# cts198859/deeprl_signal_control

Hardware: AMD Instinct MI355X
Metric: env-steps/s (agents x envs x sim-steps/s), large_grid MA2C (higher is better)
Workload: dtype f32; 1 GPU; large_grid 5x5 (25 agents), MA2C LSTM policy (neighbour fingerprint gather), 1024 env instances per GPU; step = 120 control steps (x5 sim-steps) of every instance + 1 A2C update (BPTT, clip, RMSProp); envs_per_gpu=1024, n_step=120, agents=25, parallelism=env-sharded x1, live_vehicles=window mean over the timed region

## Files before the change

deeprl_signal_control_amd/csrc/tsc_model.hip:

```cpp
#include "tsc_common.h"
#include "tsc_gemm.h"
#include "../../include/tsc.h"

#include <cstdlib>
#include <type_traits>
#include <vector>

namespace {

using tsc::f32x16;
using tsc::f32x4;
using tsc::GemmArgs;

constexpr int kOut = 8;
constexpr int kL = 64;
constexpr int kG4 = 4 * kL;

struct Layout {
    int G, A, SMAX, AMAX, H;
    int NZ, fc;
    long long stride, oW1, ob1, oWx, oWh, obl, oWo, obo;
};

__device__ __forceinline__ float sigmoidf_(float x) {
// ... 805 lines not shown
#pragma unroll
        for (int k = 0; k < kOut; ++k) {
            const float pj = __shfl(pim, row0 + k, 64);
            if (k < na) sacc += (double)pj;
            if (k == km) mine = sacc;
        }
        const long long idx = (long long)(e0 + hr) * lay.A + a;
        const double uu = uniform01(seed, step, (unsigned long long)idx);
        const bool below = hc < 8 && km < na && uu < mine / sacc;
        const unsigned long long bal = __ballot(below);
        const unsigned rowbits = (unsigned)((bal >> row0) & 0xFFull);
        const int ans = rowbits ? __ffs((int)rowbits) - 1 : na - 1;
        if (e0 + hr < E) {
            if (hc < 8 && km < lay.AMAX) pi_out[idx * lay.AMAX + km] = pim;
            if (hc == 0) {
                v_out[idx] = vv + hbv;
                if (action_out) action_out[idx] = ans;
            }
        }
    }
}


constexpr int kXLd = 68;
constexpr size_t policy_fwd_fused_lds(int H) { return sizeof(float) * ((size_t)(H + 64) * kXLd + kL * kOut + kOut + 8); }

__global__ void __launch_bounds__(256, 2)
policy_fwd_fused_kernel(const float *__restrict__ params, Layout lay, const int *__restrict__ n_act,
                        const float *__restrict__ obs, const uint8_t *__restrict__ done, float *state, int advance,
                        int E, int n_tiles, float *__restrict__ pi_out, float *__restrict__ v_out, int *action_out,
                        unsigned long long seed, unsigned long long step, long long *dbg,
                        int tslot, long long Ntot, float *X1c, float *Zc, float *Hhc, float *Ccc, float *Hpc,
                        const float *__restrict__ Wg) {
    extern __shared__ __attribute__((aligned(16))) char smem_raw[];
    float *XH = (float *)smem_raw;
    const bool stamp = dbg && blockIdx.x == 8 && threadIdx.x == 0;
    int nstamp = 0;
#define FSTAMP() do { if (stamp) dbg[nstamp++] = clock64(); } while (0)
    if (dbg && threadIdx.x == 0) dbg[64 + 2 * blockIdx.x] = wall_clock64();
    FSTAMP();
    const int b = blockIdx.x, xcd = b & 7, sidx = b >> 3;
    const int g = xcd + 8 * (sidx / n_tiles), tile = sidx % n_tiles;
    if (g >= lay.G) return;
    const int a = g >> 1, tower = g & 1, e0 = tile * 64, H = lay.H, SMAX = lay.SMAX;
    float *Hs = XH + H * kXLd;
    const float *P = params + (long long)g * lay.stride;
    const int tid = threadIdx.x, lane = tid & 63, wave = tid >> 6, li = lane & 31, kh = lane >> 5;

    const int r0 = 32 * (wave & 1), j0 = 32 * (wave >> 1), j = j0 + li;
    const int q4 = SMAX >> 2, AS = lay.A * SMAX, nct = H >> 5;
    const float *W1 = P + lay.oW1, *b1 = P + lay.ob1;
    float4 ov[4];
    int om[4], ok4[4];
#pragma unroll
    for (int q = 0; q < 4; ++q) {
        int idx = tid + 256 * q;
        om[q] = -1;
        if (idx < 64 * q4) om[q] = idx / q4; else idx = 64 * q4 - 1;
        const int m = idx / q4;
        ok4[q] = (idx % q4) * 4;
        const int e = e0 + m < E ? e0 + m : E - 1;
        ov[q] = *reinterpret_cast<const float4 *>(obs + (long long)e * AS + a * SMAX + ok4[q]);
    }
    float bw0[32];
    {
        const int ct = wave < nct ? wave : nct - 1;
        const unsigned wb = (unsigned)(ct * 32 + li) * 4u;
#pragma unroll
        for (int s2 = 0; s2 < 32; ++s2) {
            const int kr = 2 * s2 + kh < SMAX ? 2 * s2 + kh : SMAX - 1;
            bw0[s2] = ldg(W1, wb + (unsigned)(kr * H) * 4u);
        }
    }
    float *WoS = XH + (H + 64) * kXLd;
    if (tid < (kL * kOut + kOut) / 4)
        *reinterpret_cast<float4 *>(WoS + 4 * tid) = *reinterpret_cast<const float4 *>(P + lay.oWo + 4 * tid);
    float c[16], h0v[16];
    int erow[16];
    {
        const float *stb = state + (long long)g * E * 2 * kL;
#pragma unroll
        for (int r = 0; r < 16; ++r) {
            erow[r] = r0 + (r & 3) + 8 * (r >> 2) + 4 * kh;
            const int e = e0 + erow[r] < E ? e0 + erow[r] : E - 1;
            const float keep = 1.0f - (float)done[e];
            const unsigned ob = (unsigned)(e * 2 * kL + j) * 4u;
            c[r] = ldg(stb, ob) * keep; h0v[r] = ldg(stb, ob + kL * 4u) * keep;
        }
    }
#pragma unroll
    for (int q = 0; q < 4; ++q)
        if (om[q] >= 0) {
            Hs[(ok4[q] + 0) * kXLd + om[q]] = ov[q].x; Hs[(ok4[q] + 1) * kXLd + om[q]] = ov[q].y;
            Hs[(ok4[q] + 2) * kXLd + om[q]] = ov[q].z; Hs[(ok4[q] + 3) * kXLd + om[q]] = ov[q].w;
        }
    for (int idx = tid; idx < (64 - SMAX) * 64; idx += 256) Hs[(SMAX + (idx >> 6)) * kXLd + (idx & 63)] = 0.f;
    __syncthreads();
    FSTAMP();
    {
        float bw1[32];
        {
            const int ct = wave + 4 < nct ? wave + 4 : nct - 1;
            const unsigned wb = (unsigned)(ct * 32 + li) * 4u;
#pragma unroll
            for (int s2 = 0; s2 < 32; ++s2) {
                const int kr = 2 * s2 + kh < SMAX ? 2 * s2 + kh : SMAX - 1;
                bw1[s2] = ldg(W1, wb + (unsigned)(kr * H) * 4u);
            }
        }
        auto tile = [&](const float *bw, int ct) {
            f32x16 acc0, acc1;
#pragma unroll
            for (int r = 0; r < 16; ++r) { acc0[r] = 0.f; acc1[r] = 0.f; }
            const int col = ct * 32 + li;
#pragma unroll
            for (int s2 = 0; s2 < 32; ++s2) {
                const float a0 = Hs[(2 * s2 + kh) * kXLd + li], a1 = Hs[(2 * s2 + kh) * kXLd + 32 + li];
                acc0 = __builtin_amdgcn_mfma_f32_32x32x2f32(a0, bw[s2], acc0, 0, 0, 0);
                acc1 = __builtin_amdgcn_mfma_f32_32x32x2f32(a1, bw[s2], acc1, 0, 0, 0);
            }
            const float bias = b1[col];
            int eb1 = e0;
            asm volatile("" : "+v"(eb1));
#pragma unroll
            for (int r = 0; r < 16; ++r) {
                const int row = (r & 3) + 8 * (r >> 2) + 4 * kh;
                float v0 = acc0[r] + bias, v1 = acc1[r] + bias;
                v0 = v0 > 0.f ? v0 : 0.f; v1 = v1 > 0.f ? v1 : 0.f;
                XH[col * kXLd + row] = v0;
                XH[col * kXLd + 32 + row] = v1;
                if (tslot >= 0) {
                    const long long nb = (long long)g * Ntot + (long long)tslot * E + eb1;
                    if (eb1 + row < E) st_stream(X1c + ((nb + row) * H + col), v0);
                    if (eb1 + 32 + row < E) st_stream(X1c + ((nb + 32 + row) * H + col), v1);
                }
            }
        };
        if (wave < nct) tile(bw0, wave);
        if (wave + 4 < nct) tile(bw1, wave + 4);
    }
    __syncthreads();
    FSTAMP();
    int eb15 = e0;
    asm volatile("" : "+v"(eb15));
#pragma unroll
    for (int r = 0; r < 16; ++r) {
        Hs[j * kXLd + erow[r]] = h0v[r];
        if (tslot >= 0 && eb15 + erow[r] < E)
            st_stream(Hpc + (((long long)g * Ntot + (long long)tslot * E + eb15 + erow[r]) * kL + j), h0v[r]);
    }
    __syncthreads();
    FSTAMP();
    f32x16 acc[4];
    {
        const float *bl = P + lay.obl;
#pragma unroll
        for (int q = 0; q < 4; ++q) {
            const float bv = bl[64 * q + j];
#pragma unroll
            for (int r = 0; r < 16; ++r) acc[q][r] = bv;
        }
        const float *B = Wg + (long long)g * (H + 64) * kG4;
        constexpr int CS = 8;
        const int nchunk = (H + 64) / (2 * CS);
        const unsigned bb = (unsigned)(kh * kG4 + 4 * j) * 4u;
        float bA[CS][4], bB[CS][4];
        auto loadB = [&](float (*dst)[4], int chunk) {
            const float *src = B + (long long)chunk * (2 * CS * kG4);
#pragma unroll
            for (int s2 = 0; s2 < CS; ++s2) {
                const float4 w4 = ldg((const float4 *)src, bb + s2 * (2u * kG4 * 4u));
                dst[s2][0] = w4.x; dst[s2][1] = w4.y; dst[s2][2] = w4.z; dst[s2][3] = w4.w;
            }
        };
        auto compute = [&](float (*bv)[4], int chunk) {
            const float *As = XH + (chunk * 2 * CS + kh) * kXLd + r0 + li;
#pragma unroll
            for (int s2 = 0; s2 < CS; ++s2) {
                const float av = As[(2 * s2) * kXLd];
#pragma unroll
                for (int q = 0; q < 4; ++q) acc[q] = __builtin_amdgcn_mfma_f32_32x32x2f32(av, bv[s2][q], acc[q], 0, 0, 0);
            }
        };
        loadB(bA, 0);
        for (int ch = 0; ch < nchunk; ch += 2) {
            loadB(bB, ch + 1);
            compute(bA, ch);
            loadB(bA, ch + 2 < nchunk ? ch + 2 : nchunk - 1);
            compute(bB, ch + 1);
        }
    }
    FSTAMP();
    __syncthreads();
    FSTAMP();
    int row_base = e0;
    asm volatile("" : "+v"(row_base));
#pragma unroll
    for (int r = 0; r < 16; ++r) {
        const int e = row_base + erow[r];
        const float ig = sigmoidf_(acc[0][r]), fg = sigmoidf_(acc[1][r]);
        const float og = sigmoidf_(acc[2][r]), ug = tanhf_(acc[3][r]);
        const float cn = fg * c[r] + ig * ug;
        const float hn = og * tanhf_(cn);
        if (advance && e < E) {
            float *st = state + ((long long)g * E + e) * 2 * kL;
            st[j] = cn; st[kL + j] = hn;
        }
        if (tslot >= 0 && e < E) {
            const long long n = (long long)g * Ntot + (long long)tslot * E + e;
            st_stream(Zc + (n * kG4 + j), ig); st_stream(Zc + (n * kG4 + 64 + j), fg); st_stream(Zc + (n * kG4 + 128 + j), og); st_stream(Zc + (n * kG4 + 192 + j), ug);
            st_stream(Ccc + (n * kL + j), cn); st_stream(Hhc + (n * kL + j), hn);
        }
        XH[j * kXLd + erow[r]] = hn;
    }
    __syncthreads();
    FSTAMP();
    float *LG = XH + 64 * kXLd;
    {
        const float *Wo = WoS, *bo = WoS + kL * kOut;
        const int e = tid & 63, k0 = 2 * (tid >> 6);
        float s0 = 0.f, s1 = 0.f;
#pragma unroll 8
        for (int jj = 0; jj < kL; ++jj) {
            const float h = XH[jj * kXLd + e];
            s0 += h * Wo[jj * kOut + k0];
            s1 += h * Wo[jj * kOut + k0 + 1];
        }
        LG[e * kOut + k0] = s0 + bo[k0];
        LG[e * kOut + k0 + 1] = s1 + bo[k0 + 1];
    }
    __syncthreads();
    if (tid < 64 && e0 + tid < E) {
        const long long idx = (long long)(e0 + tid) * lay.A + a;
        const float *lg = LG + tid * kOut;
        if (tower == 0) {
            const int na = n_act[a];
            float mx = -INFINITY;
            for (int k = 0; k < na; ++k) mx = fmaxf(mx, lg[k]);
            float pk[kOut], sum = 0.f;
#pragma unroll
            for (int k = 0; k < kOut; ++k) { pk[k] = k < na ? expf(lg[k] - mx) : 0.f; sum += pk[k]; }
            float pn[kOut];
#pragma unroll
            for (int k = 0; k < kOut; ++k) pn[k] = pk[k] / sum;
            for (int k = 0; k < lay.AMAX; ++k) pi_out[idx * lay.AMAX + k] = k < kOut ? pn[k] : 0.f;
            if (action_out) action_out[idx] = sample_action(pn, na, seed, step, idx);
        } else {
            v_out[idx] = lg[0];
        }
    }
    FSTAMP();
    if (stamp) dbg[63] = nstamp;
    if (dbg && threadIdx.x == 0) dbg[64 + 2 * blockIdx.x + 1] = wall_clock64();
#undef FSTAMP
}

constexpr int kWsLdx = 36;
constexpr int kWsLdg = 33;
constexpr int kWsBuf = 8;
constexpr size_t policy_fwd_ws_lds(int H, int SMAX) {
    return sizeof(float) * ((size_t)32 * (H + 64 + 4) + 64 * kWsLdx + (size_t)kL * kWsLdg + (size_t)kG4 * kWsLdg + 528 +
                            (kWsBuf + 2) * 32 * kOut + (size_t)SMAX * H);
}

template <int KS2>
__global__ void __launch_bounds__(512, 1)
policy_fwd_ws_kernel(const float *__restrict__ params, Layout lay, const int *__restrict__ n_act,
                     const float *__restrict__ obs, const uint8_t *__restrict__ done, float *state, int advance,
                     int E, int S, float *__restrict__ pi_out, float *__restrict__ v_out, int *action_out,
                     unsigned long long seed, unsigned long long step,
                     int tslot, long long Ntot, float *X1c, float *Zc, float *Hhc, float *Ccc, float *Hpc,
                     long long *dbg, const float *__restrict__ Wr, const int *__restrict__ kr, int dbg_tid, const int *__restrict__ wgmap) {
    constexpr int H = 2 * KS2 - 64, NCT = H / 32;
    static_assert((32 * (H / 4)) % 512 == 0 || (32 * (H / 4)) % 512 == 256, "X1 store: duplicates come from 256 lanes below");
    const bool stamp = dbg && blockIdx.x == 0 && (int)threadIdx.x == dbg_tid;
    int nstamp = 0;
#define WSTAMP() do { if (stamp && nstamp < 60) dbg[nstamp++] = clock64(); } while (0)
    WSTAMP();
    extern __shared__ __attribute__((aligned(16))) char smem_raw[];
    constexpr int LDK = H + 64 + 4;
    float *XH = (float *)smem_raw;
    float *Hs = XH + 32 * LDK;
    float *Hn = Hs + 64 * kWsLdx;
    float *Gz = Hn + kL * kWsLdg;
    float *WoS = Gz + kG4 * kWsLdg;
    float *LG = WoS + 528;
    float *LGp = LG + kWsBuf * 32 * kOut;
    float *W1s = LGp + 2 * 32 * kOut;
    int g = blockIdx.x % lay.G, sp = blockIdx.x / lay.G;
    if (wgmap) {
        const int gs = wgmap[blockIdx.x];
        if (gs < 0) return;
        g = gs >> 8; sp = gs & 255;
    }
    const int n_half = (E + 15) / 16;
    const int eb = 16 * (int)((long long)n_half * sp / S);
    const int Ee = min(E, 16 * (int)((long long)n_half * (sp + 1) / S));
    const int nt = (Ee - eb + 31) / 32;
    const bool last_half = Ee - (eb + 32 * (nt - 1)) <= 16;
    const int a = g >> 1, tower = g & 1, SMAX = lay.SMAX;
    const float *P = params + (long long)g * lay.stride;
    const int tid = threadIdx.x, lane = tid & 63, wave = tid >> 6, li = lane & 31;
    const int col = 32 * wave + li;
    {
        const int tot = SMAX * H / 4;
        const float4 *src = reinterpret_cast<const float4 *>(P + lay.oW1);
        for (int base = tid; base < tot; base += 8 * 512) {
            float4 wq[8];
#pragma unroll
            for (int q = 0; q < 8; ++q) { const int i = base + 512 * q; wq[q] = src[i < tot ? i : tot - 1]; }
#pragma unroll
            for (int q = 0; q < 8; ++q) { const int i = base + 512 * q; if (i < tot) reinterpret_cast<float4 *>(W1s)[i] = wq[q]; }
        }
    }
    const float blc = P[lay.obl + col];
    const float b1c = wave < NCT ? P[lay.ob1 + col] : 0.f;
    if (tid < (kL * kOut + kOut) / 4)
        *reinterpret_cast<float4 *>(WoS + 4 * tid) = *reinterpret_cast<const float4 *>(P + lay.oWo + 4 * tid);
    const int q4 = SMAX >> 2, AS = lay.A * SMAX;
    const bool ob_on = tid < 32 * q4;
    const int om = ob_on ? tid / q4 : 0, ok4 = ob_on ? (tid % q4) * 4 : 0;
    const int ce = tid >> 4, cu = (tid & 15) * 4;
    float *stb = state + (long long)g * E * 2 * kL;
    const float *obs_a = obs + a * SMAX;
    auto fetch_obs = [&](int e0) {
        const unsigned e = (unsigned)(e0 + om < Ee ? e0 + om : Ee - 1);
        return *reinterpret_cast<const float4 *>(obs_a + (e * (unsigned)AS + (unsigned)ok4));
    };
    auto fetch_state = [&](int e0, int off) {
        const unsigned e = (unsigned)(e0 + ce < Ee ? e0 + ce : Ee - 1);
        return *reinterpret_cast<const float4 *>(stb + (e * (unsigned)(2 * kL) + (unsigned)(off + cu)));
    };
    auto fetch_keep = [&](int e0) { return 1.0f - (float)done[(unsigned)(e0 + ce < Ee ? e0 + ce : Ee - 1)]; };
    float4 ov = make_float4(0.f, 0.f, 0.f, 0.f), c4 = ov, h4 = ov;
    float keep = 0.f;
    if (eb >= Ee) return;
    if (dbg && threadIdx.x == 0) dbg[64 + 2 * blockIdx.x] = wall_clock64();
    ov = fetch_obs(eb); c4 = fetch_state(eb, 0); h4 = fetch_state(eb, kL); keep = fetch_keep(eb);
    float bwg[KS2];
    {
        const float4 *src4 = reinterpret_cast<const float4 *>(Wr) + ((long long)(g * 8 + wave) * (KS2 / 4)) * 64 + lane;
#pragma unroll
        for (int j4 = 0; j4 < KS2 / 4; ++j4) {
            const float4 w4 = src4[(long long)j4 * 64];
            bwg[4 * j4] = w4.x; bwg[4 * j4 + 1] = w4.y; bwg[4 * j4 + 2] = w4.z; bwg[4 * j4 + 3] = w4.w;
        }
    }
    auto emit = [&](int e0p, int nbuf) {
        if (tid >= 32 * nbuf || e0p + tid >= Ee) return;
        const long long idx = (long long)(e0p + tid) * lay.A + a;
        const float *lg = LG + tid * kOut;
        if (tower == 0) {
            const int na = n_act[a];
            float mx = -INFINITY;
            for (int k = 0; k < na; ++k) mx = fmaxf(mx, lg[k]);
            float pk[kOut], sum = 0.f;
#pragma unroll
            for (int k = 0; k < kOut; ++k) { pk[k] = k < na ? expf(lg[k] - mx) : 0.f; sum += pk[k]; }
            float pn[kOut];
#pragma unroll
            for (int k = 0; k < kOut; ++k) pn[k] = pk[k] / sum;
            for (int k = 0; k < lay.AMAX; ++k) pi_out[idx * lay.AMAX + k] = k < kOut ? pn[k] : 0.f;
            if (action_out) action_out[idx] = sample_action(pn, na, seed, step, idx);
        } else {
            v_out[idx] = lg[0];
        }
    };
    WSTAMP();
    for (int idx = tid; idx < (64 - SMAX) * 32; idx += 512) Hs[(SMAX + (idx >> 5)) * kWsLdx + (idx & 31)] = 0.f;
    int ks_lo = 0, ks_hi = (SMAX + 1) >> 1;
    if (kr && wave < NCT) { ks_lo = kr[(a * 8 + wave) * 2]; ks_hi = kr[(a * 8 + wave) * 2 + 1]; }
    auto opaque_tid = [&]() { int t_ = tid; asm volatile("" : "+v"(t_)); return t_; };
    auto stage_obs = [&]() {
        if (ob_on) {
            Hs[(ok4 + 0) * kWsLdx + om] = ov.x; Hs[(ok4 + 1) * kWsLdx + om] = ov.y;
            Hs[(ok4 + 2) * kWsLdx + om] = ov.z; Hs[(ok4 + 3) * kWsLdx + om] = ov.w;
        }
    };
    auto first_layer = [&]() {
        if (wave < NCT) {
            const int t_ = opaque_tid(), li = t_ & 31, kh = (t_ >> 5) & 1, col = 32 * (t_ >> 6) + li;
            f32x16 acc;
#pragma unroll
            for (int r = 0; r < 16; ++r) acc[r] = 0.f;
            for (int sb = ks_lo; sb < ks_hi; sb += 8) {
                float av[8], bv[8];
#pragma unroll
                for (int q = 0; q < 8; ++q) {
                    const bool on = sb + q < ks_hi;
                    const int s2 = on ? sb + q : ks_hi - 1;
                    const int row = 2 * s2 + kh < SMAX ? 2 * s2 + kh : SMAX - 1;
                    const float x = Hs[(2 * s2 + kh) * kWsLdx + li];
                    av[q] = on ? x : 0.f;
                    bv[q] = W1s[row * H + col];
                }
#pragma unroll
                for (int q4 = 0; q4 < 2; ++q4) {
                    if (sb + 4 * q4 < ks_hi) {
#pragma unroll
                        for (int q = 4 * q4; q < 4 * q4 + 4; ++q) acc = __builtin_amdgcn_mfma_f32_32x32x2f32(av[q], bv[q], acc, 0, 0, 0);
                    }
                }
            }
#pragma unroll
            for (int r = 0; r < 16; ++r) {
                const int row = (r & 3) + 8 * (r >> 2) + 4 * kh;
                float v0 = acc[r] + b1c;
                v0 = v0 > 0.f ? v0 : 0.f;
                XH[row * LDK + col] = v0;
            }
        }
    };
    float4 cm = make_float4(0.f, 0.f, 0.f, 0.f);
    auto stage_state = [&](int e0n, long long nbn, bool on) {
        const float4 hm = make_float4(h4.x * keep, h4.y * keep, h4.z * keep, h4.w * keep);
        const float4 cmn = make_float4(c4.x * keep, c4.y * keep, c4.z * keep, c4.w * keep);
        if (on) {
            const int t_ = opaque_tid(), ce = t_ >> 4, cu = (t_ & 15) * 4;
            *reinterpret_cast<float4 *>(XH + ce * LDK + H + cu) = hm;
            if (tslot >= 0 && e0n + ce < Ee) st_stream4(Hpc + nbn * kL + (unsigned)(ce * kL + cu), hm);
        }
        return cmn;
    };
    auto cell = [&](int e0c, long long nbc) {
        const int t_ = opaque_tid(), ce = t_ >> 4, cu = (t_ & 15) * 4;
        const unsigned st_lane = (unsigned)(ce * 2 * kL + cu), z_lane = (unsigned)(ce * kG4 + cu), c_lane = (unsigned)(ce * kL + cu);
        float gi[4], gf[4], go[4], gu[4], cn[4], hn[4];
        const float cin[4] = {cm.x, cm.y, cm.z, cm.w};
#pragma unroll
        for (int jj = 0; jj < 4; ++jj) {
            const int u = cu + jj;
            gi[jj] = sigmoidf_(Gz[u * kWsLdg + ce]); gf[jj] = sigmoidf_(Gz[(64 + u) * kWsLdg + ce]);
            go[jj] = sigmoidf_(Gz[(128 + u) * kWsLdg + ce]); gu[jj] = tanhf_(Gz[(192 + u) * kWsLdg + ce]);
            cn[jj] = gf[jj] * cin[jj] + gi[jj] * gu[jj];
            hn[jj] = go[jj] * tanhf_(cn[jj]);
            Hn[u * kWsLdg + ce] = hn[jj];
        }
        if (e0c + ce < Ee) {
            const float4 c4n = make_float4(cn[0], cn[1], cn[2], cn[3]), h4n = make_float4(hn[0], hn[1], hn[2], hn[3]);
            if (advance) {
                float *st = stb + (long long)e0c * 2 * kL;
                st_stream4(st + st_lane, c4n); st_stream4(st + (st_lane + kL), h4n);
            }
            if (tslot >= 0) {
                float *zr = Zc + nbc * kG4;
                st_stream4(zr + z_lane, make_float4(gi[0], gi[1], gi[2], gi[3]));
                st_stream4(zr + (z_lane + 64), make_float4(gf[0], gf[1], gf[2], gf[3]));
                st_stream4(zr + (z_lane + 128), make_float4(go[0], go[1], go[2], go[3]));
                st_stream4(zr + (z_lane + 192), make_float4(gu[0], gu[1], gu[2], gu[3]));
                st_stream4(Ccc + nbc * kL + c_lane, c4n);
                st_stream4(Hhc + nbc * kL + c_lane, h4n);
            }
        }
    };
    auto head_finish = [&](int ij) {
        if (tid < 256) {
            const int e = tid & 31, k0 = (tid >> 5) & 7, slot = ij % kWsBuf;
            LG[(slot * 32 + e) * kOut + k0] = (LGp[tid] + LGp[256 + tid]) + WoS[kL * kOut + k0];
        }
    };
    const long long nbase = (long long)g * Ntot + (long long)(tslot < 0 ? 0 : tslot) * E;
    stage_obs();
    __syncthreads();
    first_layer();
    cm = stage_state(eb, nbase + eb, true);
    ov = fetch_obs(eb + 32);
    __syncthreads();
    WSTAMP();
    auto tile = [&](auto half_tag, int it) {
        constexpr bool HALF = decltype(half_tag)::value;
        const int e0 = eb + 32 * it;
        const long long nb0 = nbase + e0;
        const bool more = it + 1 < nt;
        if (it >= 2 && (it - 2) % kWsBuf == kWsBuf - 1) emit(eb + 32 * (it - 1 - kWsBuf), kWsBuf);
        if (more) stage_obs();
        ov = fetch_obs(e0 + 64);
        c4 = fetch_state(e0 + 32, 0); h4 = fetch_state(e0 + 32, kL); keep = fetch_keep(e0 + 32);
        float hs0 = 0.f;
        {
            const int t_ = opaque_tid(), li = t_ & 31, kh = (t_ >> 5) & 1, col = 32 * (t_ >> 6) + li;
            const float *hp = Hn + (32 * (t_ >> 8)) * kWsLdg + (t_ & 31), *wp = WoS + (32 * (t_ >> 8)) * kOut + ((t_ >> 5) & 7);
            f32x16 acc;
            f32x4 acl, ach;
            float bl_ = blc;
            asm volatile("" : "+v"(bl_));
            constexpr int NJ = KS2 / 4, PER = NJ / 4, HP = NJ / 8;
            if constexpr (HALF) {
#pragma unroll
                for (int j4 = 0; j4 < NJ; ++j4) {
#pragma unroll
                    for (int c = 0; c < 2; ++c) {
                        const auto r2 = __builtin_amdgcn_permlane16_swap(__float_as_uint(bwg[4 * j4 + c]), __float_as_uint(bwg[4 * j4 + c + 2]), false, false);
                        bwg[4 * j4 + c] = __uint_as_float(r2[0]); bwg[4 * j4 + c + 2] = __uint_as_float(r2[1]);
                    }
                }
                const float bl_lo = __shfl(bl_, (t_ & 15), 64), bl_hi = __shfl(bl_, 16 + (t_ & 15), 64);
#pragma unroll
                for (int r = 0; r < 4; ++r) { acl[r] = bl_lo; ach[r] = bl_hi; }
            } else {
#pragma unroll
                for (int r = 0; r < 16; ++r) acc[r] = bl_;
            }
            const float4 *As = reinterpret_cast<const float4 *>(XH + li * LDK + 4 * kh);
            const float2 *Ah = reinterpret_cast<const float2 *>(XH + (t_ & 15) * LDK + 2 * ((t_ >> 4) & 3));
            float hv[4], wv[4];
            float4 x1q = make_float4(0.f, 0.f, 0.f, 0.f);
            unsigned x1o = 0;
            float *x1b = tslot >= 0 ? X1c + nb0 * H : X1c + (long long)lay.G * Ntot * H;
            float4 a4 = make_float4(0.f, 0.f, 0.f, 0.f);
            float2 a2 = make_float2(0.f, 0.f);
            if constexpr (HALF) a2 = Ah[0]; else a4 = As[0];
#pragma unroll
            for (int j4 = 0; j4 < NJ; ++j4) {
                float4 an = a4;
                float2 a2n = a2;
                if constexpr (HALF) a2n = Ah[4 * (j4 + 1 < NJ ? j4 + 1 : j4)];
                else an = As[2 * (j4 + 1 < NJ ? j4 + 1 : j4)];
                if (j4 % HP == 0 && j4 / HP < 8) {
#pragma unroll
                    for (int q = 0; q < 4; ++q) { hv[q] = hp[(4 * (j4 / HP) + q) * kWsLdg]; wv[q] = wp[(4 * (j4 / HP) + q) * kOut]; }
                }
                if constexpr (HALF) {
                    acl = __builtin_amdgcn_mfma_f32_16x16x4f32(a2.x, bwg[4 * j4], acl, 0, 0, 0);
                    ach = __builtin_amdgcn_mfma_f32_16x16x4f32(a2.x, bwg[4 * j4 + 2], ach, 0, 0, 0);
                    acl = __builtin_amdgcn_mfma_f32_16x16x4f32(a2.y, bwg[4 * j4 + 1], acl, 0, 0, 0);
                    ach = __builtin_amdgcn_mfma_f32_16x16x4f32(a2.y, bwg[4 * j4 + 3], ach, 0, 0, 0);
                } else {
                    acc = __builtin_amdgcn_mfma_f32_32x32x2f32(a4.x, bwg[4 * j4], acc, 0, 0, 0);
                    acc = __builtin_amdgcn_mfma_f32_32x32x2f32(a4.y, bwg[4 * j4 + 1], acc, 0, 0, 0);
                    acc = __builtin_amdgcn_mfma_f32_32x32x2f32(a4.z, bwg[4 * j4 + 2], acc, 0, 0, 0);
                    acc = __builtin_amdgcn_mfma_f32_32x32x2f32(a4.w, bwg[4 * j4 + 3], acc, 0, 0, 0);
                }
                if (j4 % HP == HP - 1 && j4 / HP < 8) {
#pragma unroll
                    for (int q = 0; q < 4; ++q) hs0 += hv[q] * wv[q];
                }
                if (j4 % PER == 3 && j4 / PER < (32 * (H / 4) + 511) / 512) {
                    int f = t_ + 512 * (j4 / PER);
                    f = f < 32 * (H / 4) ? f : f - 256;
                    int row = f / (H / 4);
                    const int c4i = f - row * (H / 4);
                    row = e0 + row < Ee ? row : Ee - 1 - e0;
                    x1q = *reinterpret_cast<const float4 *>(XH + row * LDK + 4 * c4i);
                    x1o = (unsigned)(row * H + 4 * c4i);
                }
                if (j4 % PER == 5 && j4 / PER < (32 * (H / 4) + 511) / 512 ) st_stream4(x1b + x1o, x1q);
                a4 = an; a2 = a2n;
                __builtin_amdgcn_sched_barrier(0);
            }
            if constexpr (HALF) {
                const int cl = 32 * (t_ >> 6) + (t_ & 15), rw = 4 * ((t_ >> 4) & 3);
#pragma unroll
                for (int r = 0; r < 4; ++r) { Gz[cl * kWsLdg + rw + r] = acl[r]; Gz[(cl + 16) * kWsLdg + rw + r] = ach[r]; }
            } else {
#pragma unroll
                for (int r = 0; r < 16; ++r) Gz[col * kWsLdg + (r & 3) + 8 * (r >> 2) + 4 * kh] = acc[r];
            }
            LGp[t_] = hs0;
            asm volatile("" :: "v"(ov.x), "v"(ov.y), "v"(ov.z), "v"(ov.w), "v"(c4.x), "v"(c4.y), "v"(c4.z), "v"(c4.w),
                         "v"(h4.x), "v"(h4.y), "v"(h4.z), "v"(h4.w), "v"(keep));
        }
        WSTAMP();
        __syncthreads();
        WSTAMP();
        if (it > 0) head_finish(it - 1);
        const float4 cmn = stage_state(e0 + 32, nb0 + 32, more);
#pragma unroll 1
        for (int ph = 0; ph < 2; ++ph) {
            if ((ph == 0) == (wave < 4)) { if (!HALF || wave < 4) cell(e0, nb0); }
            else if (more) first_layer();
            WSTAMP();
        }
        cm = cmn;
        __syncthreads();
        WSTAMP();
    };
    const int nt_full = last_half ? nt - 1 : nt;
    for (int it = 0; it < nt_full; ++it) tile(std::false_type{}, it);
    if (last_half) tile(std::true_type{}, nt - 1);
    {
        const int il = nt - 1;
        if (il >= 1 && (il - 1) % kWsBuf == kWsBuf - 1) emit(eb + 32 * (il - kWsBuf), kWsBuf);
        float hs0 = 0.f;
        const int e = tid & 31, k0 = (tid >> 5) & 7, hf = tid >> 8;
#pragma unroll 8
        for (int jj = 0; jj < 32; ++jj) hs0 += Hn[(32 * hf + jj) * kWsLdg + e] * WoS[(32 * hf + jj) * kOut + k0];
        LGp[tid] = hs0;
        __syncthreads();
        head_finish(il);
        __syncthreads();
        const int slot = il % kWsBuf;
        emit(eb + 32 * (il - slot), slot + 1);
    }
    if (stamp) dbg[63] = nstamp;
    if (dbg && threadIdx.x == 0) dbg[64 + 2 * blockIdx.x + 1] = wall_clock64();
#undef WSTAMP
}

__global__ void returns_kernel(const double *rew, const float *val, const uint8_t *done_all, const float *Rboot,
                               int T, int E, int A, double gamma, double rnorm, double rclip, float *Rs, float *Advs) {
    const int idx = blockIdx.x * blockDim.x + threadIdx.x;
    if (idx >= E * A) return;
    const int e = idx / A;
    double R = (double)Rboot[idx];
    for (int t = T - 1; t >= 0; --t) {
        const double d = (double)done_all[(long long)(t + 1) * E + e];
        double r = rew[(long long)t * E * A + idx];
        if (rnorm != 0.0) r = r / rnorm;
        if (rclip != 0.0) r = fmin(fmax(r, -rclip), rclip);
        R = r + gamma * R * (1.0 - d);
        const double adv = R - (double)val[(long long)t * E * A + idx];
        Rs[(long long)t * E * A + idx] = (float)R;
        Advs[(long long)t * E * A + idx] = (float)adv;
    }
}

__global__ void gae_kernel(const double *rew, const float *val, const uint8_t *done_all, const float *Rboot, int T, int E, int A,
                           double gamma, double lambda, double rnorm, double rclip, float *Rs, float *Advs) {
    const int idx = blockIdx.x * blockDim.x + threadIdx.x;
    if (idx >= E * A) return;
    const int e = idx / A;
    double vnext = (double)Rboot[idx], adv = 0.0;
    for (int t = T - 1; t >= 0; --t) {
        const double d = (double)done_all[(long long)(t + 1) * E + e];
        double r = rew[(long long)t * E * A + idx];
        if (rnorm != 0.0) r = r / rnorm;
        if (rclip != 0.0) r = fmin(fmax(r, -rclip), rclip);
        const double v = (double)val[(long long)t * E * A + idx];
        const double delta = r + gamma * vnext * (1.0 - d) - v;
        adv = delta + gamma * lambda * (1.0 - d) * adv;
        Rs[(long long)t * E * A + idx] = (float)(adv + v);
        Advs[(long long)t * E * A + idx] = (float)adv;
        vnext = v;
    }
}

__global__ void add_transition_kernel(int E, int A, int SMAX, const float *obs, const uint8_t *done_pre,
                                      const int *action, const double *reward, const float *value,
                                      const uint8_t *done_post, float *obs_t,
                                      int *act_t, double *rew_t, float *val_t, uint8_t *done_t, uint8_t *done_t1) {
    const long long i = (long long)blockIdx.x * blockDim.x + threadIdx.x;
    const long long no = (long long)E * A * SMAX;
    if (i < no && obs_t != obs) obs_t[i] = obs[i];
    if (i < (long long)E * A) {
        if (rew_t != reward) rew_t[i] = reward[i];
        if (act_t != action) act_t[i] = action[i];
        if (val_t != value) val_t[i] = value[i];
    }
    if (i < E) {
        if (done_t != done_pre) done_t[i] = done_pre[i];
        if (done_t1 != done_post) done_t1[i] = done_post[i];
    }
}

__global__ void sample_kernel(const float *pi, const int *n_act, int E, int A, int AMAX, unsigned long long seed,
                              unsigned long long step, int *action) {
    const int idx = blockIdx.x * blockDim.x + threadIdx.x;
    if (idx >= E * A) return;
    const int a = idx % A, na = n_act[a];
    const int ans = sample_action(pi + (long long)idx * AMAX, na, seed, step, idx);
    action[idx] = ans;
}

constexpr int kNormParts = 16;
__global__ void grad_norm_kernel(const float *grad, long long per_agent, double gscale, double *part) {
    __shared__ double red[256];
    const int a = blockIdx.x, c = blockIdx.y;
    const long long len = (per_agent + kNormParts - 1) / kNormParts, lo = c * len, hi = lo + len < per_agent ? lo + len : per_agent;
    const float *gp = grad + (long long)a * per_agent;
    double s = 0.0;
    for (long long i = lo + threadIdx.x; i < hi; i += 256) { const double v = (double)gp[i] * gscale; s += v * v; }
    red[threadIdx.x] = s;
    __syncthreads();
    for (int o = 128; o > 0; o >>= 1) {
        if ((int)threadIdx.x < o) red[threadIdx.x] += red[threadIdx.x + o];
        __syncthreads();
    }
    if (threadIdx.x == 0) part[a * kNormParts + c] = red[0];
}
__global__ void grad_norm_fold_kernel(const double *part, int A, double *norm2) {
    const int a = blockIdx.x * blockDim.x + threadIdx.x;
    if (a >= A) return;
    double s = 0.0;
    for (int c = 0; c < kNormParts; ++c) s += part[a * kNormParts + c];
    norm2[a] = s;
}

__global__ void rmsprop_kernel(float *w, float *ms, const float *grad, long long per_agent, long long total,
                               const double *norm2, float gscale, float clip, float lr, float alpha, float eps) {
    const long long i = (long long)blockIdx.x * blockDim.x + threadIdx.x;
    if (i >= total) return;
    const int a = (int)(i / per_agent);
    const float nrm = (float)sqrt(norm2[a]);
    float g = grad[i] * gscale;
    if (clip > 0.f) g = g * (clip / fmaxf(nrm, clip));
    const float m = alpha * ms[i] + (1.0f - alpha) * g * g;
    ms[i] = m;
    w[i] = w[i] - lr * g / sqrtf(m + eps);
}

__global__ void transpose_wx_kernel(const float *params, Layout lay, float *WxT) {
    const long long i = (long long)blockIdx.x * blockDim.x + threadIdx.x;
    const long long per = (long long)lay.H * lay.NZ;
    if (i >= per * lay.G) return;
    const int g = (int)(i / per);
    const long long r = i % per;
    const int c = (int)(r / lay.H), h = (int)(r % lay.H);
    WxT[i] = params[(long long)g * lay.stride + lay.oWx + (long long)h * lay.NZ + c];
}

__global__ void interleave_gates_kernel(const float *params, Layout lay, float *Wg) {
    const long long i = (long long)blockIdx.x * blockDim.x + threadIdx.x;
    const long long per = (long long)(lay.H + kL) * kG4;
    if (i >= per * lay.G) return;
    const long long g = i / per, r = i % per;
    const int k = (int)(r / kG4), c = (int)(r % kG4), u = c >> 2, q = c & 3;
    Wg[i] = params[g * lay.stride + lay.oWx + (long long)k * kG4 + 64 * q + u];
}

__global__ void register_order_kernel(const float *params, Layout lay, float *Wr) {
    const long long i = (long long)blockIdx.x * blockDim.x + threadIdx.x;
    const long long per = (long long)(lay.H + kL) * kG4;
    if (i >= per * lay.G) return;
    const long long g = i / per, r = i % per;
    const int c = (int)(r & 3), lane = (int)((r >> 2) & 63);
    const long long rest = r >> 8;
    const int nj = (lay.H + kL) / 8, w = (int)(rest / nj), j4 = (int)(rest % nj);
    const int k = 8 * j4 + 4 * (lane >> 5) + c, col = 32 * w + (lane & 31);
    Wr[i] = params[g * lay.stride + lay.oWx + (long long)k * kG4 + col];
}

__global__ void fill_kernel(float *p, long long n, float v) {
    const long long i = (long long)blockIdx.x * blockDim.x + threadIdx.x;
    if (i < n) p[i] = v;
}

}

typedef const float __attribute__((address_space(1))) *gfloat_p;
typedef const f32x4 __attribute__((address_space(1))) *gfloat4_p;
__device__ __forceinline__ gfloat_p uniform_ptr(const float *p) {
    const unsigned long long v = (unsigned long long)p;
    const unsigned lo = __builtin_amdgcn_readfirstlane((unsigned)v), hi = __builtin_amdgcn_readfirstlane((unsigned)(v >> 32));
    return (gfloat_p)(((unsigned long long)hi << 32) | lo);
}

constexpr long long split_rows(long long N, int S, int quantum) { return ((N + S - 1) / S + quantum - 1) / quantum * quantum; }

constexpr int kDwKc = 16, kDwKi = 64;
constexpr int kDwK = 2;
template <int NT> constexpr size_t dwxh_lds() { return sizeof(float) * 2 * kDwKi * (NT * 32 + 4); }
constexpr long long dwxh_ws_floats(int H) { return (long long)(H + kL + 1) * kG4; }

template <int NT>
__global__ void __launch_bounds__(512, 1)
dwxh_kernel(const float *__restrict__ X1, const float *__restrict__ Hp, const float *__restrict__ dZ, long long N, int G,
            int S, long long rows_per_split, float *__restrict__ ws, long long *dbg) {
    constexpr int HT = NT - 2, H = 32 * HT, KC = kDwKc, LDA = NT * 32 + 4;
    constexpr int XQ = H / 4, NX = KC * XQ;
    static_assert(NX >= 512 && NX <= 1024 && NX % 64 == 0 && KC * (kL / 4) == 256, "staging slots");
    extern __shared__ __attribute__((aligned(16))) char smem_raw[];
    float *As = (float *)smem_raw;
    const int g = blockIdx.x % G, sp = blockIdx.x / G;
    const int tid = threadIdx.x, lane = tid & 63, wave = __builtin_amdgcn_readfirstlane(tid >> 6), li = lane & 31, kh = lane >> 5;
    const int col0 = 32 * wave;
    const long long n0 = (long long)sp * rows_per_split;
    long long n1 = n0 + rows_per_split;
// ... 1306 lines not shown
```

Measured before the change: 393.5 million env-steps/s.

## Overlap kernel prologue weight loads with first-layer compute and obs fetch

Restructures the kernel prologue so the global loads for W1, Wo, the biases, the k-range bounds and the first obs/state tile are all issued together before any LDS store, with sched barriers holding that order. The per-wave recurrent weight register preload (bwg) is split: the first part is loaded up front and the rest is interleaved into a new first_layer_fill routine between its MFMA groups. The aim is to shorten the serial latency chain in the prologue by overlapping memory latency with compute. It raises register pressure (wq[8] plus bwg held live at once), and the unrolled fill loop adds code size.

```diff
diff --git a/deeprl_signal_control_amd/csrc/tsc_model.hip b/deeprl_signal_control_amd/csrc/tsc_model.hip
--- a/deeprl_signal_control_amd/csrc/tsc_model.hip
+++ b/deeprl_signal_control_amd/csrc/tsc_model.hip
@@ -1131,21 +1131,6 @@
     const float *P = params + (long long)g * lay.stride;
     const int tid = threadIdx.x, lane = tid & 63, wave = tid >> 6, li = lane & 31;
     const int col = 32 * wave + li;
-    {
-        const int tot = SMAX * H / 4;
-        const float4 *src = reinterpret_cast<const float4 *>(P + lay.oW1);
-        for (int base = tid; base < tot; base += 8 * 512) {
-            float4 wq[8];
-#pragma unroll
-            for (int q = 0; q < 8; ++q) { const int i = base + 512 * q; wq[q] = src[i < tot ? i : tot - 1]; }
-#pragma unroll
-            for (int q = 0; q < 8; ++q) { const int i = base + 512 * q; if (i < tot) reinterpret_cast<float4 *>(W1s)[i] = wq[q]; }
-        }
-    }
-    const float blc = P[lay.obl + col];
-    const float b1c = wave < NCT ? P[lay.ob1 + col] : 0.f;
-    if (tid < (kL * kOut + kOut) / 4)
-        *reinterpret_cast<float4 *>(WoS + 4 * tid) = *reinterpret_cast<const float4 *>(P + lay.oWo + 4 * tid);
     const int q4 = SMAX >> 2, AS = lay.A * SMAX;
     const bool ob_on = tid < 32 * q4;
     const int om = ob_on ? tid / q4 : 0, ok4 = ob_on ? (tid % q4) * 4 : 0;
@@ -1161,20 +1146,52 @@
         return *reinterpret_cast<const float4 *>(stb + (e * (unsigned)(2 * kL) + (unsigned)(off + cu)));
     };
     auto fetch_keep = [&](int e0) { return 1.0f - (float)done[(unsigned)(e0 + ce < Ee ? e0 + ce : Ee - 1)]; };
-    float4 ov = make_float4(0.f, 0.f, 0.f, 0.f), c4 = ov, h4 = ov;
-    float keep = 0.f;
     if (eb >= Ee) return;
     if (dbg && threadIdx.x == 0) dbg[64 + 2 * blockIdx.x] = wall_clock64();
-    ov = fetch_obs(eb); c4 = fetch_state(eb, 0); h4 = fetch_state(eb, kL); keep = fetch_keep(eb);
+    const int w1tot = SMAX * H / 4;
+    const float4 *w1src = reinterpret_cast<const float4 *>(P + lay.oW1);
+    float4 wq[8];
+#pragma unroll
+    for (int q = 0; q < 8; ++q) { const int i = tid + 512 * q; wq[q] = w1src[i < w1tot ? i : w1tot - 1]; }
+    __builtin_amdgcn_sched_barrier(0);
+    const bool wo_on = tid < (kL * kOut + kOut) / 4;
+    float4 woq = *reinterpret_cast<const float4 *>(P + lay.oWo + (wo_on ? 4 * tid : 0));
+    const float blc = P[lay.obl + col];
+    const float b1r = P[lay.ob1 + (wave < NCT ? col : 0)];
+    const bool kr_on = kr && wave < NCT;
+    const int *krp = kr_on ? kr + (a * 8 + wave) * 2 : n_act + a;
+    const int kr_lo = krp[0], kr_hi = krp[kr_on ? 1 : 0];
+    __builtin_amdgcn_sched_barrier(0);
+    float4 ov = fetch_obs(eb), c4 = fetch_state(eb, 0), h4 = fetch_state(eb, kL);
+    float keep = fetch_keep(eb);
+    __builtin_amdgcn_sched_barrier(0);
     float bwg[KS2];
-    {
-        const float4 *src4 = reinterpret_cast<const float4 *>(Wr) + ((long long)(g * 8 + wave) * (KS2 / 4)) * 64 + lane;
-#pragma unroll
-        for (int j4 = 0; j4 < KS2 / 4; ++j4) {
-            const float4 w4 = src4[(long long)j4 * 64];
-            bwg[4 * j4] = w4.x; bwg[4 * j4 + 1] = w4.y; bwg[4 * j4 + 2] = w4.z; bwg[4 * j4 + 3] = w4.w;
-        }
-    }
+    const float4 *wsrc4 = reinterpret_cast<const float4 *>(Wr) + ((long long)(g * 8 + wave) * (KS2 / 4)) * 64 + lane;
+    auto load_wq = [&](int j4) {
+        const float4 w4 = wsrc4[(long long)j4 * 64];
+        bwg[4 * j4] = w4.x; bwg[4 * j4 + 1] = w4.y; bwg[4 * j4 + 2] = w4.z; bwg[4 * j4 + 3] = w4.w;
+    };
+    constexpr int NPRE = 8;
+#pragma unroll
+    for (int j4 = 0; j4 < NPRE; ++j4) load_wq(j4);
+#pragma unroll
+    for (int q = 0; q < 8; ++q) {
+        const int i = tid + 512 * q;
+        asm volatile("" : "+v"(wq[q].x), "+v"(wq[q].y), "+v"(wq[q].z), "+v"(wq[q].w));
+        if (i < w1tot) reinterpret_cast<float4 *>(W1s)[i] = wq[q];
+    }
+    for (int base = tid + 8 * 512; base < w1tot; base += 8 * 512) {
+        float4 wr[8];
+#pragma unroll
+        for (int q = 0; q < 8; ++q) { const int i = base + 512 * q; wr[q] = w1src[i < w1tot ? i : w1tot - 1]; }
+#pragma unroll
+        for (int q = 0; q < 8; ++q) { const int i = base + 512 * q; if (i < w1tot) reinterpret_cast<float4 *>(W1s)[i] = wr[q]; }
+    }
+    asm volatile("" : "+v"(woq.x), "+v"(woq.y), "+v"(woq.z), "+v"(woq.w));
+    if (wo_on) *reinterpret_cast<float4 *>(WoS + 4 * tid) = woq;
+    const float b1c = wave < NCT ? b1r : 0.f;
+    const int ks_lo = kr_on ? kr_lo : 0, ks_hi = kr_on ? kr_hi : (SMAX + 1) >> 1;
+    for (int idx = tid; idx < (64 - SMAX) * 32; idx += 512) Hs[(SMAX + (idx >> 5)) * kWsLdx + (idx & 31)] = 0.f;
     auto emit = [&](int e0p, int nbuf) {
         if (tid >= 32 * nbuf || e0p + tid >= Ee) return;
         const long long idx = (long long)(e0p + tid) * lay.A + a;
@@ -1195,10 +1212,6 @@
             v_out[idx] = lg[0];
         }
     };
-    WSTAMP();
-    for (int idx = tid; idx < (64 - SMAX) * 32; idx += 512) Hs[(SMAX + (idx >> 5)) * kWsLdx + (idx & 31)] = 0.f;
-    int ks_lo = 0, ks_hi = (SMAX + 1) >> 1;
-    if (kr && wave < NCT) { ks_lo = kr[(a * 8 + wave) * 2]; ks_hi = kr[(a * 8 + wave) * 2 + 1]; }
     auto opaque_tid = [&]() { int t_ = tid; asm volatile("" : "+v"(t_)); return t_; };
     auto stage_obs = [&]() {
         if (ob_on) {
@@ -1229,6 +1242,56 @@
 #pragma unroll
                         for (int q = 4 * q4; q < 4 * q4 + 4; ++q) acc = __builtin_amdgcn_mfma_f32_32x32x2f32(av[q], bv[q], acc, 0, 0, 0);
                     }
+                }
+            }
+#pragma unroll
+            for (int r = 0; r < 16; ++r) {
+                const int row = (r & 3) + 8 * (r >> 2) + 4 * kh;
+                float v0 = acc[r] + b1c;
+                v0 = v0 > 0.f ? v0 : 0.f;
+                XH[row * LDK + col] = v0;
+            }
+        }
+    };
+    auto first_layer_fill = [&]() {
+        const int t_ = opaque_tid(), li = t_ & 31, kh = (t_ >> 5) & 1, col = 32 * (t_ >> 6) + li;
+        const bool fl_on = (t_ >> 6) < NCT;
+        constexpr int NQ = KS2 / 4, PER = (NQ - NPRE + 7) / 8;
+        f32x16 acc;
+#pragma unroll
+        for (int r = 0; r < 16; ++r) acc[r] = 0.f;
+#pragma unroll
+        for (int gi = 0; gi < 8; ++gi) {
+            const int sb = ks_lo + 4 * gi;
+            const bool run = fl_on && sb < ks_hi;
+            float av[4], bv[4];
+            if (run) {
+#pragma unroll
+                for (int q = 0; q < 4; ++q) {
+                    const bool on = sb + q < ks_hi;
+                    const int s2 = on ? sb + q : ks_hi - 1;
+                    const int row = 2 * s2 + kh < SMAX ? 2 * s2 + kh : SMAX - 1;
+                    const float x = Hs[(2 * s2 + kh) * kWsLdx + li];
+                    av[q] = on ? x : 0.f;
+                    bv[q] = W1s[row * H + col];
+                }
+            }
+#pragma unroll
+            for (int k = 0; k < PER; ++k) if (NPRE + gi * PER + k < NQ) load_wq(NPRE + gi * PER + k);
+            if (run) {
+#pragma unroll
+                for (int q = 0; q < 4; ++q) acc = __builtin_amdgcn_mfma_f32_32x32x2f32(av[q], bv[q], acc, 0, 0, 0);
+            }
+        }
+        if (fl_on) {
+            for (int sb = ks_lo + 32; sb < ks_hi; sb += 4) {
+#pragma unroll
+                for (int q = 0; q < 4; ++q) {
+                    const bool on = sb + q < ks_hi;
+                    const int s2 = on ? sb + q : ks_hi - 1;
+                    const int row = 2 * s2 + kh < SMAX ? 2 * s2 + kh : SMAX - 1;
+                    const float x = Hs[(2 * s2 + kh) * kWsLdx + li];
+                    acc = __builtin_amdgcn_mfma_f32_32x32x2f32(on ? x : 0.f, W1s[row * H + col], acc, 0, 0, 0);
                 }
             }
 #pragma unroll
@@ -1290,8 +1353,9 @@
     };
     const long long nbase = (long long)g * Ntot + (long long)(tslot < 0 ? 0 : tslot) * E;
     stage_obs();
+    WSTAMP();
     __syncthreads();
-    first_layer();
+    first_layer_fill();
     cm = stage_state(eb, nbase + eb, true);
     ov = fetch_obs(eb + 32);
     __syncthreads();
```

New measurement: 394.7 million env-steps/s, median of 3. Within noise of the previous version (+0.3%).
